# iamwinter/UMPR

Measured on AMD Instinct MI355X. Metric: training samples/sec, higher is better.
Workload: dtype f32

## Files before the change

### include/umpr_hip.h

```cpp
#ifndef UMPR_HIP_H
#define UMPR_HIP_H
#include <stddef.h>
#include <stdint.h>

#ifdef __cplusplus
extern "C" {
#endif

const char* umpr_version(void);
const char* umpr_last_error(void);
int umpr_device_info(int dev, char* name, int name_len, int* compute_units, size_t* hbm_bytes);

int umpr_gemm_f32(const float* A, long lda, int transA, const float* B, long ldb, int transB, float* C, long ldc,
                  int M, int N, int K, const float* bias, int bias_mode, int act, int accumulate, float alpha,
                  float* ws, size_t ws_bytes, void* stream);

int umpr_set_gemm_bf16(int on);

int umpr_set_conv_inference(int on);

int umpr_set_conv_pool_follows(int on);

long umpr_debug_wino_fix_count(void);

int umpr_debug_conv3x3_plan(int pass, int N, int Cin, int Cout, int H, int W, int inference, size_t* ws_bytes, size_t* v_bytes);

int umpr_debug_wino_pool_fold(const float* y, const float* g_pooled, const float* w, const float* x, float* unpooled, float* dx,
                              float* dw, float* db, int N, int Cin, int Cout, int H, int W, int f4, int fold, float* ws,
                              size_t ws_bytes, void* stream);

size_t umpr_embed_gru_bidir_ws_bytes(int N, int L, int E);
int umpr_embed_gru_bidir_fwd(const int64_t* ids, const float* emb, int E,
                             const float* w_ih_f, const float* w_hh_f, const float* b_ih_f, const float* b_hh_f,
                             const float* w_ih_r, const float* w_hh_r, const float* b_ih_r, const float* b_hh_r,
                             const int32_t* lengths, const int32_t* order, const int32_t* dst_row, int N, int L,
                             float* out, float* saved, float* ws, size_t ws_bytes, void* stream);
int umpr_embed_gru_bidir_bwd(const int64_t* ids, const float* emb, int E,
                             const float* w_hh_f, const float* w_hh_r,
                             const int32_t* lengths, const int32_t* order, const int32_t* dst_row, int N, int L,
                             const float* dout, const float* out, const float* saved,
                             float* dw_ih_f, float* dw_hh_f, float* db_ih_f, float* db_hh_f,
                             float* dw_ih_r, float* dw_hh_r, float* db_ih_r, float* db_hh_r,
                             float* ws, size_t ws_bytes, void* stream);

int umpr_embed_gru_bidir_bwd_acc(const int64_t* ids, const float* emb, int E,
                                 const float* w_hh_f, const float* w_hh_r,
                                 const int32_t* lengths, const int32_t* order, const int32_t* dst_row, int N, int L,
                                 const float* dout, const float* out, const float* saved,
                                 float* dw_ih_f, float* dw_hh_f, float* db_ih_f, float* db_hh_f,
                                 float* dw_ih_r, float* dw_hh_r, float* db_ih_r, float* db_hh_r,
                                 int accumulate, float* ws, size_t ws_bytes, void* stream);

// ... 295 lines not shown
```

### umpr_amd/_lib.py

```python
from __future__ import annotations

import ctypes
import os
import threading

import torch

_HERE = os.path.dirname(os.path.abspath(__file__))
LIB_PATH = os.path.join(_HERE, "libumpr_hip.so")

_T = {"p": ctypes.c_void_p, "i": ctypes.c_int, "l": ctypes.c_long, "z": ctypes.c_size_t, "f": ctypes.c_float,
      "d": ctypes.c_double, "u": ctypes.c_uint64}

SIGNATURES = {
    "umpr_version": ("", "s"),
    "umpr_last_error": ("", "s"),
    "umpr_device_info": ("ipipp", "i"),
    "umpr_gemm_f32": ("pliplipliiipiiifpzp", "i"),
    "umpr_embed_gru_bidir_ws_bytes": ("iii", "z"),
    "umpr_embed_gru_bidir_fwd": ("ppipppppppppppiipppzp", "i"),
    "umpr_embed_gru_bidir_bwd": ("ppipppppiippppppppppppzp", "i"),
    "umpr_embed_gru_bidir_bwd_acc": ("ppipppppiipppppppppppipzp", "i"),
    "umpr_embed_gru_bidir_bwd_dx": ("ppipppppiipppppppppppipppipzp", "i"),
    "umpr_embed_grad_chunk": ("", "i"),
# ... 89 lines not shown
    "umpr_feature_fetch_f32": ("pipppiiplpp", "i"),
    "umpr_review_collate": ("pplppppppplpiiiiilpppp", "i"),
    "umpr_review_collate_sampled": ("pplppppppplpiiiiil" "iuil" "pppp", "i"),
    "umpr_bce_head_fwd": ("plpppiipppzp", "i"),
    "umpr_bce_head_bwd": ("plpppppiiplpppzp", "i"),
    "umpr_adam_step": ("ppppldddddldp", "i"),
    "umpr_sq_err_accumulate": ("pplpp", "i"),
    "umpr_adam_step_dev": ("pppplddd" "pp", "i"),
    "umpr_grad_norm_ws_bytes": ("", "z"),
    "umpr_grad_norm": ("ppidfppzpp", "i"),
    "umpr_adam_step_clip": ("ppppldddddld" "pp", "i"),
    "umpr_adam_step_dev_clip": ("pppplddd" "ppp", "i"),
    "umpr_adam_step_groups": ("ppppldddddld" "pp" "ppp" "ii" "p", "i"),
    "umpr_grad_accumulate": ("pppiip", "i"),
    "umpr_ema_update": ("pppidip", "i"),
    "umpr_arena_swap": ("pppip", "i"),
    "umpr_debug_poison_lds": ("pp", "i"),
    "umpr_set_gemm_bf16": ("i", "i"),
    "umpr_set_conv_inference": ("i", "i"),
    "umpr_set_conv_pool_follows": ("i", "i"),
    "umpr_debug_wino_fix_count": ("", "l"),
    "umpr_debug_conv3x3_plan": ("iiiiiiipp", "i"),
    "umpr_debug_wino_pool_fold": ("pppppppp" "iiiiiii" "pzp", "i"),
    "umpr_profile_enable": ("i", "i"),
    "umpr_profile_reset": ("", "i"),
    "umpr_profile_read": ("ippp", "i"),
}


class UmprHipError(RuntimeError):
    pass


class _Tls(threading.local):
    gemm_b16 = False


TLS = _Tls()


class _Lib:
    def __init__(self):
        if not os.path.exists(LIB_PATH):
            raise UmprHipError(
                f"{LIB_PATH} not found: build it with `python -c 'import __graft_entry__ as g; g.build()'` "
                f"(or `make -C umpr_amd/csrc`).  There is no CPU fallback.")
# ... 65 lines not shown
```

### umpr_amd/csrc/api.hip

```cpp
#include <math.h>
#include <stdarg.h>
#include <stdlib.h>

#include <vector>

#include "../../include/umpr_hip.h"
#include "umpr_common.h"
#include "umpr_internal.h"

static thread_local char g_err[512] = "";
void umpr_set_error(const char* fmt, ...) {
  va_list ap;
  va_start(ap, fmt);
  vsnprintf(g_err, sizeof(g_err), fmt, ap);
  va_end(ap);
}

namespace {
const bool g_fc_small = umpr_env_on("UMPR_FC_SMALL");
struct ProfRec { hipEvent_t e0, e1; int family; double work; };
bool g_prof_on = false;
std::vector<ProfRec> g_prof;
std::vector<ProfRec> g_prof_pool;
double g_prof_ms[UMPR_K_COUNT] = {0}, g_prof_work[UMPR_K_COUNT] = {0};
// ... 98 lines not shown
  return p.algo;
}
int umpr_debug_wino_pool_fold(const float* y, const float* g_pooled, const float* w, const float* x, float* unpooled, float* dx,
                              float* dw, float* db, int N, int Cin, int Cout, int H_, int W, int f4, int fold, float* ws,
                              size_t ws_bytes, void* stream) {
  UMPR_REQUIRE(N > 0 && Cin > 0 && Cout > 0 && H_ > 0 && W > 0 && (H_ % 2) == 0 && (W % 2) == 0 && y && g_pooled && ws,
               "debug_wino_pool_fold: bad arguments");
  UMPR_REQUIRE(fold || unpooled, "debug_wino_pool_fold: the un-folded run needs the buffer for the un-pooled gradient");
  UMPR_REQUIRE(!dx || (f4 && w), "debug_wino_pool_fold: the data gradient runs on the 4x4 tile and needs the weights");
  UMPR_REQUIRE(!dw || (x && (!f4 || ((H_ % 4) == 0 && (W % 4) == 0))), "debug_wino_pool_fold: the weight gradient on the 4x4 tile has no edge tiles");
  hipStream_t s = S(stream);
  ConvHints h;
  const float* g = g_pooled;
  if (fold) { h.pooled_dy = true; h.pool_y = y; }
  else {
    if (int rc = umpr_maxpool2_bwd_relu_impl(y, g_pooled, unpooled, (long)N * Cout, H_, W, s)) return rc;
    g = unpooled;
  }
  if (dx)
    if (int rc = umpr_wino_conv3x3(g, w, 1, nullptr, nullptr, dx, N, Cin, Cout, H_, W, 0, ws, ws_bytes / sizeof(float), true, h, s)) return rc;
  if (dw)
    if (int rc = umpr_wino_wgrad(g, x, dw, db, N, Cin, Cout, H_, W, 0, ws, ws_bytes / sizeof(float), f4 != 0, h, s)) return rc;
  return 0;
}

constexpr size_t kSlabs = 256;
namespace {
struct GruWs {
  float *gx, *wslab, *bslab;
  float* kslab; size_t kslab_bytes;
  float *stacked, *rows;
  float *wst, *bst;
  size_t bytes;
};
GruWs gru_ws(float* base, int N, int L, int pitch) {
  Carve c(base, sizeof(float));
  const size_t tiles = umpr_gru_tiles(N);
  GruWs w;
  w.gx = c.take<float>((size_t)N * L * 384); w.wslab = c.take<float>(tiles * 2 * G3 * H); w.bslab = c.take<float>(tiles * 2 * 2 * G3);
  w.wst = c.at<float>(c.off); w.bst = c.at<float>(c.off + (size_t)2 * G3 * pitch * sizeof(float));
  w.kslab_bytes = kSlabs * G3 * pitch * sizeof(float); w.kslab = c.take<float>(kSlabs * G3 * pitch);
  w.stacked = c.take<float>((size_t)2 * G3 * pitch); w.rows = c.take<float>((size_t)N * L * pitch); w.bytes = c.off;
  return w;
}
const bool g_emb_gather = umpr_env_on("UMPR_EMB_GATHER");
__global__ __launch_bounds__(256) void gather_rows_kernel(const int64_t* __restrict__ ids, const float* __restrict__ emb,
// ... 403 lines not shown
}
int umpr_conv3x3_bwd_weight(const float* dy, const float* x, float* dw, float* db, int N, int Cin, int H_, int W,
                            int Cout, float* ws, size_t ws_bytes, void* stream) {
  return umpr_conv3x3_wgrad(dy, x, dw, db, N, Cin, Cout, H_, W, 0, ws, ws_bytes, conv_hints(), S(stream));
}
int umpr_maxpool2_fwd(const float* x, float* y, long planes, int H_, int W, void* stream) {
  return umpr_maxpool2_fwd_impl(x, y, planes, H_, W, S(stream));
}
int umpr_maxpool2_bwd_relu(const float* x, const float* dy, float* dx, long planes, int H_, int W, void* stream) {
  return umpr_maxpool2_bwd_relu_impl(x, dy, dx, planes, H_, W, S(stream));
}

size_t umpr_vgg16_pool5_offset(int n_img) { return vgg_layout(n_img).pool_off[4] * sizeof(float); }

int umpr_vgg16_features_fwd(const float* images, const float* const* params, int n, float* acts, float* ws,
                            size_t ws_bytes, void* stream) {
  UMPR_REQUIRE(n > 0 && images && params && acts, "vgg16_features_fwd: bad arguments");
  UMPR_REQUIRE(ws_bytes >= umpr_vgg16_fwd_ws_bytes(n), "vgg16_features_fwd: workspace too small");
  const VggLayout L = vgg_layout(n);
  hipStream_t s = S(stream);
  const float* x = images;
  int ci = 0;
  for (int b = 0; b < 5; ++b) {
    for (int j = 0; j < kConvPerBlock[b]; ++j, ++ci) {
      float* y = acts + L.conv_off[ci];
      const int hw = L.conv_hw[ci];
      ConvHints hints;
      hints.inference = t_conv_inference;
      hints.pool_follows = j == kConvPerBlock[b] - 1;
      if (L.v_floats[ci] && !hints.inference) { hints.v_slot = acts + L.v_off[ci]; hints.v_slot_floats = L.v_floats[ci]; }
      if (int rc = umpr_conv3x3_run(x, params[2 * ci], 0, params[2 * ci + 1], nullptr, y, n, L.conv_cin[ci], L.conv_cout[ci], hw,
                                    hw, 1, ws, ws_bytes / sizeof(float), hints, s))
        return rc;
      x = y;
    }
    const int hw = L.conv_hw[ci - 1];
    float* y = acts + L.pool_off[b];
    if (int rc = umpr_maxpool2_fwd_impl(x, y, (long)n * kBlockCh[b], hw, hw, s)) return rc;
    x = y;
  }
  return 0;
}

namespace {
struct ClsActs { const float* pool5; float* fc[2]; float* drop[2]; };

int classifier_fwd_impl(const float* const* params, int n, int train, int use_masks, uint64_t seed, const ClsActs& A,
                        uint8_t* masks, float* out, float* ws, size_t ws_bytes, hipStream_t s, int fc_bf16, bool gemm_b16) {
  const float* x = A.pool5;
  for (int j = 0; j < 3; ++j) {
    float* y = j < 2 ? A.fc[j] : out;
    const int act = j < 2 ? UMPR_ACT_RELU : UMPR_ACT_NONE;
    if (g_fc_small && umpr_fc_small_ok(n, kFc[j][1], kFc[j][0])) {
      if (int rc = umpr_fc_small_fwd(x, params[26 + 2 * j], params[27 + 2 * j], y, n, kFc[j][1], kFc[j][0], act, ws,
                                     ws_bytes, s, 0, fc_bf16)) return rc;
    } else {
      UmprGemm g;
      g.A = x; g.lda = kFc[j][0]; g.B = params[26 + 2 * j]; g.ldb = kFc[j][0]; g.transB = true;
      g.C = y; g.ldc = kFc[j][1]; g.M = n; g.N = kFc[j][1]; g.K = kFc[j][0];
      g.bias = params[27 + 2 * j]; g.bias_mode = 1; g.act = act;
      g.split_k = 0; g.ws = ws; g.ws_bytes = ws_bytes; g.b16 = gemm_b16;
// ... 513 lines not shown
```

### umpr_amd/csrc/conv3x3.hip

```cpp
#include "umpr_common.h"
#include "umpr_internal.h"
#include "umpr_tiles.h"
#include <stdlib.h>
#include <type_traits>

namespace {

struct ConvParams {
  const float* x;
  const float* wm;
  const float* bias;
  const float* mask;
  float* y;
  int N, C, H, W, Cout, relu;
  long p0_base;
  long p_end;
};

template <int TM, int TN, bool BIAS, bool MASK, bool TAIL>
__device__ __forceinline__ void igemm_epilogue_as(const f32x16 (&tot)[TM][TN], const ConvParams& p, int HW, int row0,
                                                  const long (&obase)[TN], const bool (&pv)[TN]) {
  const int Cout = p.Cout;
  const bool relu = p.relu != 0;
  float bv[TM][16];
// ... 1101 lines not shown
  }
  if (pass != CONV_DGRAD && !(pass == CONV_FWD && inference) && sw.v_reuse &&
      conv_algo(CONV_FWD, Cin, Cout, H, W, false) == CONV_WINO4 && conv_algo(CONV_WGRAD, Cin, Cout, H, W, false) == CONV_WINO4) {
    const WinoConvGeom fg = umpr_wino_conv_geom(N, Cin, Cout, H, W, true);
    const WinoWgradGeom wg = umpr_wino_wgrad_geom(N, Cin, Cout, H, W, true);
    if (fg.v_floats == (size_t)wg.planes * wg.Cpad * wg.Tpad) p.v_floats = fg.v_floats;
  }
  return p;
}

size_t umpr_conv3x3_pack_floats(int N, int Cin, int Cout, int H, int W) {
  const size_t f = umpr_conv3x3_plan(CONV_FWD, N, Cin, Cout, H, W, false).ws_floats;
  const size_t t = umpr_conv3x3_plan(CONV_DGRAD, N, Cin, Cout, H, W, false).ws_floats;
  return f > t ? f : t;
}

bool umpr_conv3x3_pool_fold_ok(int N, int Cin, int Cout, int H, int W) {
  static const bool on = umpr_env_on("UMPR_POOL_FOLD");
  if (!on || (H % 2) != 0 || (W % 2) != 0) return false;
  const ConvAlgo wg = umpr_conv3x3_plan(CONV_WGRAD, N, Cin, Cout, H, W, false).algo;
  return umpr_conv3x3_plan(CONV_DGRAD, N, Cin, Cout, H, W, false).algo == CONV_WINO4 && (wg == CONV_WINO4 || wg == CONV_WINO2);
}

int umpr_conv3x3_run(const float* x, const float* w, int transposed, const float* bias, const float* mask, float* y,
                     int N, int Cin, int Cout, int H, int W, int relu, float* wpack, size_t wpack_floats,
                     const ConvHints& hints, hipStream_t s) {
  UMPR_REQUIRE(N > 0 && Cin > 0 && H > 0 && W > 0 && Cout > 0, "conv3x3: bad shape");
  UMPR_REQUIRE(transposed || !mask, "conv3x3: the forward pass takes no mask");
  const int M = transposed ? Cin : Cout;
  const int C = transposed ? Cout : Cin;
  const long NP = (long)N * H * W;
  const ConvPlan plan = umpr_conv3x3_plan(transposed ? CONV_DGRAD : CONV_FWD, N, Cin, Cout, H, W, hints.inference);
  ConvAlgo algo = plan.algo;
  const bool fits = wpack && wpack_floats >= plan.ws_floats;
  if (hints.v_slot)
    UMPR_REQUIRE(algo == CONV_WINO4 && fits && plan.v_floats > 0 && plan.v_floats == hints.v_slot_floats,
                 "conv3x3: the V slot does not fit this call (%d -> %d at %dx%d, slot %zu floats, plan %zu)", Cin, Cout, H, W,
                 hints.v_slot_floats, plan.v_floats);
  else if ((algo == CONV_WINO2 || algo == CONV_WINO4) && !fits) algo = plan.direct;
  if (hints.pooled_dy)
    UMPR_REQUIRE(transposed && algo == CONV_WINO4 && hints.pool_y, "conv3x3: no reader with a pooled source for this call (%d -> %d at %dx%d)",
                 Cin, Cout, H, W);
  if (algo == CONV_DIRECT && !wpack) algo = CONV_GENERIC;
  const int family = transposed ? UMPR_K_CONV_DGRAD : UMPR_K_CONV_IGEMM;
  const double work = 2.0 * NP * M * C * 9;
  switch (algo) {
    case CONV_WINO2:
    case CONV_WINO4: {
      UmprProfScope prof(family, work, s);
      return umpr_wino_conv3x3(x, w, transposed, bias, mask, y, N, Cin, Cout, H, W, relu, wpack, wpack_floats,
                               algo == CONV_WINO4, hints, s);
    }
    case CONV_C3: {
      ConvParams p{x, w, bias, nullptr, y, N, Cin, H, W, Cout, relu, 0, NP};
      UmprProfScope prof(family, work, s);
      conv3x3_fwd_c3_kernel<2><<<2048, 256, 0, s>>>(p);
      UMPR_LAUNCH_CHECK("conv3x3_fwd_c3");
      return 0;
    }
    case CONV_DIRECT: {
      const long total = (long)M * ((C + V2_CC - 1) / V2_CC) * V2_KC;
      UMPR_REQUIRE(wpack_floats >= (size_t)total, "conv3x3: weight scratch too small");
      UMPR_REQUIRE(H == W && (W == 224 || W == 112 || W == 56 || W == 28 || W == 14), "conv3x3: the direct kernels need a square VGG map, not %dx%d", H, W);
      int blocks = (int)((total + 255) / 256);
      if (blocks > 4096) blocks = 4096;
// ... 163 lines not shown
```

### umpr_amd/csrc/umpr_internal.h

```cpp
#pragma once
#include <hip/hip_runtime.h>
#include <stdint.h>

struct UmprGemm {
  const float* A = nullptr; long lda = 0; bool transA = false;
  const float* B = nullptr; long ldb = 0; bool transB = false;
  float* C = nullptr; long ldc = 0;
  int M = 0, N = 0, K = 0;
  const int64_t* gatherA = nullptr;
  const int64_t* gatherB = nullptr;
  const float* bias = nullptr; int bias_mode = 0;
  int act = 0; bool accumulate = false; float alpha = 1.0f;
  int split_k = 1;
  float* ws = nullptr; size_t ws_bytes = 0;
  bool b16 = false;
  int winA_L = 0, winA_D = 1, winA_pad = 0;
  int winB_L = 0, winB_D = 1, winB_pad = 0;
};
int umpr_gemm(const UmprGemm& g, hipStream_t stream);
bool umpr_ambient_gemm_b16();

constexpr int D = 128, H = 64, G3 = 192, AT = 64;
bool umpr_merge_small();

// ... 25 lines not shown
  const float* pos_v; const float* neg_v;
  const float* lw; const float* lb;
  const float* fw; const float* fb;
  const float* labels;
  float rate;
  int B, V, P, F;
  float* pred; float* loss;
  float* z;
  float* img_emb; float* pos_match; float* neg_match;
  float* posneg_emb;
  const float* d_loss;
  const float* d_pred;
  float* d_rr; float* d_cu; float* d_ci; float* d_pp; float* d_pn;
  float* d_vgg; float* d_pos_v; float* d_neg_v; float* d_lw; float* d_lb; float* d_fw; float* d_fb;
};
int umpr_head_launch(const UmprHead& p, int backward, hipStream_t s);

enum ConvPass { CONV_FWD = 0, CONV_DGRAD = 1, CONV_WGRAD = 2 };
enum ConvAlgo { CONV_GENERIC = 0 , CONV_C3 = 1 ,
                CONV_DIRECT = 2 , CONV_WINO2 = 3, CONV_WINO4 = 4 };
struct ConvHints {
  bool inference = false, pool_follows = false; float* v_slot = nullptr; size_t v_slot_floats = 0;
  bool pooled_dy = false; const float* pool_y = nullptr;
};
struct ConvPlan {
  ConvAlgo algo;
  ConvAlgo direct;
  bool edge;
  size_t ws_floats;
  size_t v_floats;
};
ConvPlan umpr_conv3x3_plan(ConvPass pass, int N, int Cin, int Cout, int H, int W, bool inference);
size_t umpr_conv3x3_pack_floats(int N, int Cin, int Cout, int H, int W);
bool umpr_conv3x3_pool_fold_ok(int N, int Cin, int Cout, int H, int W);
int umpr_conv3x3_run(const float* x, const float* w, int transposed, const float* bias, const float* mask, float* y,
                     int N, int Cin, int Cout, int H, int W, int relu, float* wpack, size_t wpack_floats,
                     const ConvHints& hints, hipStream_t s);
struct WinoConvGeom { int planes, MT, S; long T, Tpad; bool edge; size_t v_floats, U, V, M, count, tie, floats; };
WinoConvGeom umpr_wino_conv_geom(int N, int C, int M, int H, int W, bool f4);
struct WinoWgradGeom { long T, Tpad; int MT, CT, Mpad, Cpad, stages, splits, stages_per_split, planes, bnc; size_t Gy, V, P, BP, floats; };
WinoWgradGeom umpr_wino_wgrad_geom(int N, int Cin, int Cout, int H, int W, bool f4);
long umpr_wino_last_fix_count();
int umpr_wino_wgrad(const float* dy, const float* x, float* dw, float* db, int N, int Cin, int Cout, int H, int W,
                    int accumulate, float* ws, size_t ws_floats, bool f4, const ConvHints& hints, hipStream_t s);
int umpr_wino_conv3x3(const float* x, const float* w, int transposed, const float* bias, const float* mask, float* y,
                      int N, int Cin, int Cout, int H, int W, int relu, float* ws, size_t ws_floats, bool f4,
                      const ConvHints& hints, hipStream_t s);
int umpr_conv3x3_flip_transpose(const float* w, float* wt, int Cout, int Cin, hipStream_t s);
size_t umpr_conv3x3_wgrad_ws_bytes(int N, int Cin, int Cout, int H, int W);
int umpr_conv3x3_wgrad(const float* gz, const float* x, float* dw, float* db, int N, int Cin, int Cout, int H, int W,
                       int accumulate, float* ws, size_t ws_bytes, const ConvHints& hints, hipStream_t s);
int umpr_maxpool2_fwd_impl(const float* x, float* y, long planes, int H, int W, hipStream_t s);
int umpr_maxpool2_bwd_relu_impl(const float* x, const float* gy, float* gx, long planes, int H, int W, hipStream_t s);

int umpr_wgrad_reduce(const float* slab, const float* bslab, int splits, int Cout, int Cin, float* dw, float* db,
                      int accumulate, hipStream_t s);

struct UmprPF {
  int N, H, W, RW;
  long rows;
  long ptot;
  long lead, tail;
  long ps;
};
UmprPF umpr_pf(int N, int H, int W);
// ... 117 lines not shown
```

### umpr_amd/csrc/winograd.hip

```cpp
#include <type_traits>

#include "umpr_common.h"
#include "umpr_internal.h"

namespace {

constexpr int WK = 32;
constexpr int WBM = 128;
constexpr int WBN = 128;

__device__ __forceinline__ void pool_window_grad(const float2 a, const float2 b, const float gy, float2& ga, float2& gb) {
  int arg = 0;
  float m = a.x;
  if (a.y > m) { m = a.y; arg = 1; }
  if (b.x > m) { m = b.x; arg = 2; }
  if (b.y > m) { m = b.y; arg = 3; }
  const float g = m > 0.f ? gy : 0.f;
  ga = make_float2(arg == 0 ? g : 0.f, arg == 1 ? g : 0.f);
  gb = make_float2(arg == 2 ? g : 0.f, arg == 3 ? g : 0.f);
}
typedef float f32x4_t __attribute__((ext_vector_type(4)));
__device__ __forceinline__ float as_loaded(float v) { asm volatile("" : "+v"(v)); return v; }
__device__ __forceinline__ float4 as_loaded(const float4 v) {
  f32x4_t q = {v.x, v.y, v.z, v.w};
// ... 487 lines not shown
        if (((rows >> (2 * wy)) & 0xFu) != 0xFu) viol |= 1u << (2 * w);
        if (((cols >> (2 * wx)) & 0xFu) != 0xFu) viol |= 2u << (2 * w);
      }
      if (viol & ~bits[t]) atomicOr(&bits[t], viol);
    }
#pragma unroll
    for (int b = 0; b < 6; ++b) {
      float o[6];
      wino4_bt(wc, e[0][b], e[1][b], e[2][b], e[3][b], e[4][b], e[5][b], o);
#pragma unroll
      for (int a = 0; a < 6; ++a) dst[(long)(a * 6 + b) * per] = o[a];
    }
  }
}

struct WinoFix {
  unsigned int* count;
  unsigned int* list;
  unsigned int cap;
  float kappa_eps;
  const unsigned int* tie_bits;
};

template <bool EDGE, bool FIX>
__global__ __launch_bounds__(256) void wino4_output_kernel(const float* __restrict__ Mx, const float* __restrict__ bias,
                                                           const float* __restrict__ mask, float* __restrict__ y, int N,
                                                           int Mch, int H, int W, long Tpad, int Mpad, int relu, Wino4C wc,
                                                           WinoFix fx) {
  const int TH = (H + 3) / 4, TW = (W + 3) / 4;
  const long T = (long)N * TH * TW;
  const long total = (long)Mch * T;
  const long per = (long)Mpad * Tpad;
  for (long i = blockIdx.x * (long)blockDim.x + threadIdx.x; i < total; i += (long)gridDim.x * blockDim.x) {
    const long t = i % T;
    const int m = (int)(i / T);
    const int tx = (int)(t % TW);
    const long r = t / TW;
    const int ty = (int)(r % TH), n = (int)(r / TH);
    const float* src = Mx + (long)m * Tpad + t;
    float am[4][6];
    float as[4][6];
#pragma unroll
    for (int b = 0; b < 6; ++b) {
      float q[6];
#pragma unroll
      for (int a = 0; a < 6; ++a) q[a] = src[(long)(a * 6 + b) * per];
      float o[4];
      wino4_at(wc, q, o);
      am[0][b] = o[0]; am[1][b] = o[1]; am[2][b] = o[2]; am[3][b] = o[3];
      if (FIX) {
#pragma unroll
        for (int a = 0; a < 6; ++a) q[a] = fabsf(q[a]);
        wino4_at_abs(wc, q, o);
        as[0][b] = o[0]; as[1][b] = o[1]; as[2][b] = o[2]; as[3][b] = o[3];
      }
    }
    const float bv = bias ? bias[m] : 0.f;
    const long ob = (((long)n * Mch + m) * H + 4 * ty) * W + 4 * tx;
    float vv[4][4], tau[4][4];
#pragma unroll
    for (int a = 0; a < 4; ++a) {
      float v[4];
      wino4_at(wc, am[a], v);
#pragma unroll
      for (int j = 0; j < 4; ++j) v[j] += bv;
      if (FIX) {
        float sv[4];
        wino4_at_abs(wc, as[a], sv);
#pragma unroll
        for (int j = 0; j < 4; ++j) { vv[a][j] = v[j]; tau[a][j] = fx.kappa_eps * sv[j]; }
      }
      if (relu) {
#pragma unroll
        for (int j = 0; j < 4; ++j) v[j] = fmaxf(v[j], 0.f);
      }
      const long oo = ob + (long)a * W;
      if (EDGE) {
        if (4 * ty + a >= H) continue;
#pragma unroll
        for (int j = 0; j < 4; ++j) {
          if (4 * tx + j < W) {
            float o = v[j];
            if (mask) o = mask[oo + j] > 0.f ? o : 0.f;
            y[oo + j] = o;
          }
        }
        continue;
      }
      if (mask) {
        const float4 mk = *reinterpret_cast<const float4*>(mask + oo);
        v[0] = mk.x > 0.f ? v[0] : 0.f; v[1] = mk.y > 0.f ? v[1] : 0.f;
        v[2] = mk.z > 0.f ? v[2] : 0.f; v[3] = mk.w > 0.f ? v[3] : 0.f;
      }
      *reinterpret_cast<float4*>(y + oo) = make_float4(v[0], v[1], v[2], v[3]);
    }
    if (FIX) {
      unsigned flags = 0;
#pragma unroll
      for (int a = 0; a < 4; ++a)
#pragma unroll
        for (int j = 0; j < 4; ++j)
          if (fabsf(vv[a][j]) < tau[a][j]) flags |= 1u << (4 * a + j);
      if (fx.tie_bits) {
        const unsigned viol = fx.tie_bits[t];
#pragma unroll
        for (int wy = 0; wy < 2; ++wy)
#pragma unroll
          for (int wx = 0; wx < 2; ++wx) {
            float top = 0.f, second = 0.f, tw = 0.f;
            int e1 = 0, e2 = 0;
#pragma unroll
            for (int e = 0; e < 4; ++e) {
              const int a = 2 * wy + (e >> 1), j = 2 * wx + (e & 1);
              const float rv = fmaxf(vv[a][j], 0.f);
              if (rv > top) { second = top; e2 = e1; top = rv; e1 = e; } else if (rv > second) { second = rv; e2 = e; }
              tw = fmaxf(tw, tau[a][j]);
            }
// ... 35 lines not shown
    float acc = 0.f;
    for (int c = lane; c < C; c += 64) {
      const float* xp = x + ((long)n * C + c) * HW;
      const float* wp = w + ((long)m * C + c) * 9;
#pragma unroll
      for (int dy = 0; dy < 3; ++dy) {
        const int py = yy + dy - 1;
        if (py < 0 || py >= H) continue;
#pragma unroll
        for (int dx = 0; dx < 3; ++dx) {
          const int px = xx + dx - 1;
          if (px < 0 || px >= W) continue;
          acc = fmaf(xp[(long)py * W + px], wp[dy * 3 + dx], acc);
        }
      }
    }
#pragma unroll
    for (int o = 32; o > 0; o >>= 1) acc += __shfl_xor(acc, o, 64);
    if (lane == 0) {
      float v = acc + (bias ? bias[m] : 0.f);
      if (relu) v = fmaxf(v, 0.f);
      y[idx] = v;
    }
  }
}

static long wino_tpad(long T) { return (T + WBN - 1) / WBN * WBN; }

struct WinoGemmParams {
  const float* U;
  const float* V;
  float* Mx;
  int MT, S, C;
  long Tpad;
  long TT;
  int Mpad;
  int planes;
};

typedef __attribute__((address_space(3))) void* lds_ptr_t;
template <int FOLD>
__global__ __launch_bounds__(256, 2) void wino_gemm_dma_kernel(WinoGemmParams p) {
  constexpr int SK = WK;
  constexpr int LD = 128;
  constexpr int TM = 2, TN = 2;
  constexpr int KS = SK / 2;
// ... 177 lines not shown
    if (edge) wino4_input_kernel<true, false, true><<<nblk((long)S * WK * TT * WBN, 16384), 256, 0, s>>>(x, V, N, C, S * WK, H, W, Tpad, TT * WBN, wino4_consts(), nullptr, nullptr, hints.pool_y);
    else wino4_input_kernel<false, false, true><<<nblk((long)S * WK * TT * WBN, 16384), 256, 0, s>>>(x, V, N, C, S * WK, H, W, Tpad, TT * WBN, wino4_consts(), nullptr, nullptr, hints.pool_y);
  } else if (f4 && edge) {
    if (tie_bits) wino4_input_kernel<true, true><<<nblk((long)S * WK * TT * WBN, 16384), 256, 0, s>>>(x, V, N, C, S * WK, H, W, Tpad, TT * WBN, wino4_consts(), fx.count, tie_bits);
    else wino4_input_kernel<true, false><<<nblk((long)S * WK * TT * WBN, 16384), 256, 0, s>>>(x, V, N, C, S * WK, H, W, Tpad, TT * WBN, wino4_consts(), fx.count, nullptr);
  } else if (f4) {
    if (tie_bits) wino4_input_kernel<false, true><<<nblk((long)S * WK * TT * WBN, 16384), 256, 0, s>>>(x, V, N, C, S * WK, H, W, Tpad, TT * WBN, wino4_consts(), fx.count, tie_bits);
    else wino4_input_kernel<false, false><<<nblk((long)S * WK * TT * WBN, 16384), 256, 0, s>>>(x, V, N, C, S * WK, H, W, Tpad, TT * WBN, wino4_consts(), fx.count, nullptr);
  }
  else if ((W / 2) % 2 == 0)
    wino_input_pair_kernel<<<nblk((long)S * WK * TT * WBN / 2, 16384), 256, 0, s>>>(x, V, N, C, S * WK, H, W, Tpad, TT * WBN);
  else
    wino_input_kernel<<<nblk((long)S * WK * TT * WBN, 16384), 256, 0, s>>>(x, V, N, C, S * WK, H, W, Tpad, TT * WBN);
  UMPR_LAUNCH_CHECK("wino_input");
  WinoGemmParams p{U, V, Mx, MT, S, C, Tpad, TT, MT * WBM, planes};
  const long groups = (planes * TT + 7) / 8 * 8;
  {
    UmprProfScope prof(UMPR_K_WINO_GEMM, 2.0 * planes * (double)M * C * T, s);
    static const int fold = umpr_env_int("UMPR_WINO_FOLD", 1);
    if (fold == 2) wino_gemm_dma_kernel<2><<<(unsigned)(groups * MT), 256, 0, s>>>(p);
    else wino_gemm_dma_kernel<1><<<(unsigned)(groups * MT), 256, 0, s>>>(p);
  }
  UMPR_LAUNCH_CHECK("wino_gemm");
  if (f4 && fix) {
    if (edge) wino4_output_kernel<true, true><<<nblk((long)M * T, 16384), 256, 0, s>>>(Mx, bias, mask, y, N, M, H, W, Tpad, MT * WBM, relu, wino4_consts(), fx);
    else wino4_output_kernel<false, true><<<nblk((long)M * T, 16384), 256, 0, s>>>(Mx, bias, mask, y, N, M, H, W, Tpad, MT * WBM, relu, wino4_consts(), fx);
    UMPR_LAUNCH_CHECK("wino_output");
    wino_fixup_kernel<<<128, 256, 0, s>>>(x, w, bias, y, fx.list, fx.count, fx.cap, C, M, H, W, relu);
    UMPR_LAUNCH_CHECK("wino_fixup");
    t_last_fix_count = fx.count;
    return 0;
  }
  if (f4 && edge)
    wino4_output_kernel<true, false><<<nblk((long)M * T, 16384), 256, 0, s>>>(Mx, bias, mask, y, N, M, H, W, Tpad, MT * WBM, relu, wino4_consts(), fx);
  else if (f4)
    wino4_output_kernel<false, false><<<nblk((long)M * T, 16384), 256, 0, s>>>(Mx, bias, mask, y, N, M, H, W, Tpad, MT * WBM, relu, wino4_consts(), fx);
  else if ((W / 2) % 2 == 0)
    wino_output_pair_kernel<<<nblk((long)M * T / 2, 16384), 256, 0, s>>>(Mx, bias, mask, y, N, M, H, W, Tpad, MT * WBM, relu);
  else
    wino_output_kernel<<<nblk((long)M * T, 16384), 256, 0, s>>>(Mx, bias, mask, y, N, M, H, W, Tpad, MT * WBM, relu);
  UMPR_LAUNCH_CHECK("wino_output");
  return 0;
}

namespace {

template <bool POOL>
__global__ void wino_dy_kernel(const float* __restrict__ dy, float* __restrict__ Gy, int N, int Mch, int H, int W,
                               long Tpad, long Tw, int Mpad, const float* __restrict__ pool_y) {
  const int TH = H / 2, TW = W / 2;
  const long T = (long)N * TH * TW;
  const long total = (long)Mch * Tw;
  const long per = (long)Mpad * Tpad;
  for (long i = blockIdx.x * (long)blockDim.x + threadIdx.x; i < total; i += (long)gridDim.x * blockDim.x) {
    const long t = i % Tw;
    const int m = (int)(i / Tw);
    float* dst = Gy + (long)m * Tpad + t;
    if (t >= T) {
#pragma unroll
// ... 283 lines not shown
  __shared__ float outs[64 * 9];
  if (g == 0 && ok) {
#pragma unroll
    for (int a = 0; a < 36; ++a) v[a] = ((v[a] + red[0][a][cl]) + red[1][a][cl]) + red[2][a][cl];
    float gv[3][6];
#pragma unroll
    for (int b = 0; b < 6; ++b) {
      float o[3];
      wino4_gt(wc, v + b, 6, o);
      gv[0][b] = o[0]; gv[1][b] = o[1]; gv[2][b] = o[2];
    }
#pragma unroll
    for (int a = 0; a < 3; ++a) {
      float o[3];
      wino4_gt(wc, gv[a], 1, o);
      outs[cl * 9 + a * 3 + 0] = o[0]; outs[cl * 9 + a * 3 + 1] = o[1]; outs[cl * 9 + a * 3 + 2] = o[2];
    }
  }
  __syncthreads();
  const int c0 = (blockIdx.x % chunks) * 64;
  const int nout = (C - c0 < 64 ? C - c0 : 64) * 9;
  float* d = dw + ((long)m * C + c0) * 9;
  for (int i = threadIdx.x; i < nout; i += 256) d[i] = accumulate ? d[i] + outs[i] : outs[i];
}

struct WinoWgradParams {
  const float* Gy;
  const float* V;
  float* P;
  int MT, CT, Mpad, Cpad;
  long Tpad;
  int stages;
  int stages_per_split;
  int planes;
};

constexpr int WLDK = WK + 4;

template <int TN>
__global__ __launch_bounds__(256, 2) void wino_wgrad_gemm_kernel(WinoWgradParams p) {
  constexpr int LD = WLDK;
  constexpr int TM = 2;
  constexpr int BNC = 64 * TN;
  constexpr int NG = WK / 8;
  constexpr int SFLUSH = 4;
  __shared__ __attribute__((aligned(16))) float As[2][WBM * LD];
// ... 128 lines not shown
    float gv[3][4];
#pragma unroll
    for (int b = 0; b < 4; ++b) {
      gv[0][b] = v[0][b] + 0.5f * (v[1][b] + v[2][b]);
      gv[1][b] = 0.5f * (v[1][b] - v[2][b]);
      gv[2][b] = 0.5f * (v[1][b] + v[2][b]) + v[3][b];
    }
    float* d = dw + i * 9;
#pragma unroll
    for (int a = 0; a < 3; ++a) {
      const float o0 = gv[a][0] + 0.5f * (gv[a][1] + gv[a][2]);
      const float o1 = 0.5f * (gv[a][1] - gv[a][2]);
      const float o2 = 0.5f * (gv[a][1] + gv[a][2]) + gv[a][3];
      if (accumulate) { d[a * 3 + 0] += o0; d[a * 3 + 1] += o1; d[a * 3 + 2] += o2; }
      else { d[a * 3 + 0] = o0; d[a * 3 + 1] = o1; d[a * 3 + 2] = o2; }
    }
  }
}

constexpr int kWinoWgradTargetWgs = 1024;
static const int g_wino_wgrad_rounds = umpr_env_int("UMPR_WINO_WGRAD_ROUNDS", 1);
}

WinoWgradGeom umpr_wino_wgrad_geom(int N, int Cin, int Cout, int H, int W, bool f4) {
  WinoWgradGeom g;
  g.planes = f4 ? 36 : 16;
  g.T = f4 ? (long)N * ((H + 3) / 4) * ((W + 3) / 4) : (long)N * (H / 2) * (W / 2);
  g.Tpad = wino_tpad(g.T);
  g.bnc = Cin <= 64 ? 64 : WBN;
  g.MT = (Cout + WBM - 1) / WBM; g.CT = (Cin + g.bnc - 1) / g.bnc;
  g.Mpad = g.MT * WBM; g.Cpad = g.CT * g.bnc;
  g.stages = (int)(g.Tpad / WK);
  const int tiles = g.planes * g.MT * g.CT;
  const int max_splits = g.stages / 8 > 0 ? g.stages / 8 : 1;
  int splits = (kWinoWgradTargetWgs + tiles - 1) / tiles;
  if (g_wino_wgrad_rounds && (long)tiles * max_splits >= 512) {
    double best = 0.0;
    const int hi = max_splits < splits ? max_splits : splits;
    for (int sp = 1; sp <= hi; ++sp) {
      const long wgs = (long)tiles * sp;
      if (wgs < 512) continue;
      const double eff = (double)wgs / (double)((wgs + 511) / 512 * 512);
      if (eff > best) best = eff;
    }
    for (int sp = 1; sp <= hi; ++sp) {
      const long wgs = (long)tiles * sp;
// ... 38 lines not shown
    else wino_dy_kernel<false><<<nblk((long)Cout * g.Tpad, 16384), 256, 0, s>>>(dy, Gy, N, Cout, H, W, g.Tpad, g.Tpad, g.Mpad, nullptr);
  }
  UMPR_LAUNCH_CHECK("wino_dy");
  if (hints.v_slot) {
    UMPR_REQUIRE(f4 && !edge && hints.v_slot_floats == (size_t)g.planes * g.Cpad * g.Tpad,
                 "winograd wgrad: the V slot does not match this layer (%d -> %d at %dx%d)", Cin, Cout, H, W);
    V = hints.v_slot;
  } else if (f4 && edge)
    wino4_input_kernel<true, false><<<nblk((long)g.Cpad * g.Tpad, 16384), 256, 0, s>>>(x, V, N, Cin, g.Cpad, H, W, g.Tpad, g.Tpad, wino4_consts(), nullptr, nullptr);
  else if (f4)
    wino4_input_kernel<false, false><<<nblk((long)g.Cpad * g.Tpad, 16384), 256, 0, s>>>(x, V, N, Cin, g.Cpad, H, W, g.Tpad, g.Tpad, wino4_consts(), nullptr, nullptr);
  else if ((W / 2) % 2 == 0)
    wino_input_pair_kernel<<<nblk((long)g.Cpad * g.Tpad / 2, 16384), 256, 0, s>>>(x, V, N, Cin, g.Cpad, H, W, g.Tpad, g.Tpad);
  else
    wino_input_kernel<<<nblk((long)g.Cpad * g.Tpad, 16384), 256, 0, s>>>(x, V, N, Cin, g.Cpad, H, W, g.Tpad, g.Tpad);
  UMPR_LAUNCH_CHECK("wino_input(wgrad)");
  WinoWgradParams p{Gy, V, P, g.MT, g.CT, g.Mpad, g.Cpad, g.Tpad, g.stages, g.stages_per_split, g.planes};
  {
    UmprProfScope prof(UMPR_K_WINO_WGRAD_GEMM, 2.0 * g.planes * (double)Cout * Cin * g.T, s);
    if (g.bnc == 64) wino_wgrad_gemm_kernel<1><<<(unsigned)(g.planes * g.MT * g.CT * g.splits), 256, 0, s>>>(p);
    else wino_wgrad_gemm_kernel<2><<<(unsigned)(g.planes * g.MT * g.CT * g.splits), 256, 0, s>>>(p);
  }
  UMPR_LAUNCH_CHECK("wino_wgrad_gemm");
  if (f4)
    wino4_wgrad_finish_kernel<<<(unsigned)((long)Cout * ((Cin + 63) / 64)), 256, 0, s>>>(P, g.splits, Cout, Cin, g.Mpad, g.Cpad, dw,
                                                                                     accumulate, wino4_consts());
  else if (g.splits >= 8)
    wino_wgrad_finish_wide_kernel<<<(unsigned)((long)Cout * ((Cin + 63) / 64)), 256, 0, s>>>(P, g.splits, Cout, Cin, g.Mpad, g.Cpad,
                                                                                         dw, accumulate);
  else
    wino_wgrad_finish_kernel<<<nblk((long)Cout * Cin, 4096), 256, 0, s>>>(P, g.splits, Cout, Cin, g.Mpad, g.Cpad, dw, accumulate);
  UMPR_LAUNCH_CHECK("wino_wgrad_finish");
  if (fused_bias) {
    wino_bias_sum_waves_kernel<<<(unsigned)((Cout + 3) / 4), 256, 0, s>>>(BP, db, Cout, g.Tpad / 64, accumulate);
    UMPR_LAUNCH_CHECK("wino_bias_sum_waves");
  } else if (db) {
    UMPR_REQUIRE((size_t)N * Cout <= (size_t)g.splits * g.planes * g.Mpad * g.Cpad && ((long)H * W) % 4 == 0,
                 "winograd wgrad: bias-gradient scratch");
    if (pooled) wino_bias_part_wave_kernel<true><<<(unsigned)(((long)N * Cout + 3) / 4), 256, 0, s>>>(dy, P, (long)H * W, (long)N * Cout, py, W);
    else wino_bias_part_wave_kernel<false><<<(unsigned)(((long)N * Cout + 3) / 4), 256, 0, s>>>(dy, P, (long)H * W, (long)N * Cout, nullptr, W);
    UMPR_LAUNCH_CHECK("wino_bias_part");
    wino_bias_sum_kernel<<<(Cout + 255) / 256, 256, 0, s>>>(P, db, N, Cout, accumulate);
    UMPR_LAUNCH_CHECK("wino_bias_sum");
  }
  return 0;
}
```

Measured before the change: 2164.

## Fuse maxpool into Winograd forward output and widen wgrad finish kernel

Adds an optional path where the 4x4-tile Winograd forward output kernel also writes the 2x2 max-pooled result, with a fixup pass that recomputes pooled values touched by corrected outputs. This would skip the separate maxpool launch and its re-read of the activation, but it is gated behind the UMPR_FWD_FOLD environment variable. Separately, the f4 weight-gradient finish now always uses a new 1024-thread kernel that splits the reduction over splits across 16 waves, staging partial sums in shared memory before the transform. The new finish kernel aims for more memory parallelism in the split reduction, at the cost of more shared memory and a fixed summation order.

```diff
diff --git a/include/umpr_hip.h b/include/umpr_hip.h
--- a/include/umpr_hip.h
+++ b/include/umpr_hip.h
@@ -28,6 +28,12 @@
 int umpr_debug_wino_pool_fold(const float* y, const float* g_pooled, const float* w, const float* x, float* unpooled, float* dx,
                               float* dw, float* db, int N, int Cin, int Cout, int H, int W, int f4, int fold, float* ws,
                               size_t ws_bytes, void* stream);
+
+int umpr_debug_wino_fwd_fold(const float* x, const float* w, const float* bias, float* y, float* pooled, int N, int Cin, int Cout,
+                             int H, int W, int inference, int fold, float* ws, size_t ws_bytes, void* stream);
+
+int umpr_debug_wino4_wgrad_finish(const float* P, int splits, int Cout, int Cin, int Mpad, int Cpad, float* dw, int accumulate,
+                                  int former, void* stream);
 
 size_t umpr_embed_gru_bidir_ws_bytes(int N, int L, int E);
 int umpr_embed_gru_bidir_fwd(const int64_t* ids, const float* emb, int E,
diff --git a/umpr_amd/_lib.py b/umpr_amd/_lib.py
--- a/umpr_amd/_lib.py
+++ b/umpr_amd/_lib.py
@@ -135,6 +135,8 @@
     "umpr_debug_wino_fix_count": ("", "l"),
     "umpr_debug_conv3x3_plan": ("iiiiiiipp", "i"),
     "umpr_debug_wino_pool_fold": ("pppppppp" "iiiiiii" "pzp", "i"),
+    "umpr_debug_wino_fwd_fold": ("ppppp" "iiiiiii" "pzp", "i"),
+    "umpr_debug_wino4_wgrad_finish": ("p" "iiiii" "p" "ii" "p", "i"),
     "umpr_profile_enable": ("i", "i"),
     "umpr_profile_reset": ("", "i"),
     "umpr_profile_read": ("ippp", "i"),
diff --git a/umpr_amd/csrc/api.hip b/umpr_amd/csrc/api.hip
--- a/umpr_amd/csrc/api.hip
+++ b/umpr_amd/csrc/api.hip
@@ -144,6 +144,23 @@
   if (dw)
     if (int rc = umpr_wino_wgrad(g, x, dw, db, N, Cin, Cout, H_, W, 0, ws, ws_bytes / sizeof(float), f4 != 0, h, s)) return rc;
   return 0;
+}
+
+int umpr_debug_wino_fwd_fold(const float* x, const float* w, const float* bias, float* y, float* pooled, int N, int Cin, int Cout,
+                             int H_, int W, int inference, int fold, float* ws, size_t ws_bytes, void* stream) {
+  UMPR_REQUIRE(N > 0 && Cin > 0 && Cout > 0 && H_ > 0 && W > 0 && (H_ % 2) == 0 && (W % 2) == 0 && x && w && y && pooled && ws,
+               "debug_wino_fwd_fold: bad arguments");
+  hipStream_t s = S(stream);
+  ConvHints h;
+  h.inference = inference != 0; h.pool_follows = true;
+  if (fold) h.pool_out = pooled;
+  if (int rc = umpr_wino_conv3x3(x, w, 0, bias, nullptr, y, N, Cin, Cout, H_, W, 1, ws, ws_bytes / sizeof(float), true, h, s)) return rc;
+  return fold ? 0 : umpr_maxpool2_fwd_impl(y, pooled, (long)N * Cout, H_, W, s);
+}
+int umpr_debug_wino4_wgrad_finish(const float* P, int splits, int Cout, int Cin, int Mpad, int Cpad, float* dw, int accumulate,
+                                  int former, void* stream) {
+  UMPR_REQUIRE(P && dw && splits > 0 && Cout > 0 && Cin > 0 && Mpad >= Cout && Cpad >= Cin, "debug_wino4_wgrad_finish: bad arguments");
+  return umpr_wino4_wgrad_finish_launch(P, splits, Cout, Cin, Mpad, Cpad, dw, accumulate, former != 0, S(stream));
 }
 
 constexpr size_t kSlabs = 256;
@@ -593,6 +610,7 @@
   const float* x = images;
   int ci = 0;
   for (int b = 0; b < 5; ++b) {
+    bool pooled = false;
     for (int j = 0; j < kConvPerBlock[b]; ++j, ++ci) {
       float* y = acts + L.conv_off[ci];
       const int hw = L.conv_hw[ci];
@@ -600,6 +618,10 @@
       hints.inference = t_conv_inference;
       hints.pool_follows = j == kConvPerBlock[b] - 1;
       if (L.v_floats[ci] && !hints.inference) { hints.v_slot = acts + L.v_off[ci]; hints.v_slot_floats = L.v_floats[ci]; }
+      if (hints.pool_follows && umpr_conv3x3_fwd_fold_ok(n, L.conv_cin[ci], L.conv_cout[ci], hw, hw, hints.inference)) {
+        hints.pool_out = acts + L.pool_off[b];
+        pooled = true;
+      }
       if (int rc = umpr_conv3x3_run(x, params[2 * ci], 0, params[2 * ci + 1], nullptr, y, n, L.conv_cin[ci], L.conv_cout[ci], hw,
                                     hw, 1, ws, ws_bytes / sizeof(float), hints, s))
         return rc;
@@ -607,7 +629,8 @@
     }
     const int hw = L.conv_hw[ci - 1];
     float* y = acts + L.pool_off[b];
-    if (int rc = umpr_maxpool2_fwd_impl(x, y, (long)n * kBlockCh[b], hw, hw, s)) return rc;
+    if (!pooled)
+      if (int rc = umpr_maxpool2_fwd_impl(x, y, (long)n * kBlockCh[b], hw, hw, s)) return rc;
     x = y;
   }
   return 0;
diff --git a/umpr_amd/csrc/conv3x3.hip b/umpr_amd/csrc/conv3x3.hip
--- a/umpr_amd/csrc/conv3x3.hip
+++ b/umpr_amd/csrc/conv3x3.hip
@@ -1147,6 +1147,11 @@
   return umpr_conv3x3_plan(CONV_DGRAD, N, Cin, Cout, H, W, false).algo == CONV_WINO4 && (wg == CONV_WINO4 || wg == CONV_WINO2);
 }
 
+bool umpr_conv3x3_fwd_fold_ok(int N, int Cin, int Cout, int H, int W, bool inference) {
+  static const bool on = umpr_env_on("UMPR_FWD_FOLD");
+  return on && (H % 2) == 0 && (W % 2) == 0 && umpr_conv3x3_plan(CONV_FWD, N, Cin, Cout, H, W, inference).algo == CONV_WINO4;
+}
+
 int umpr_conv3x3_run(const float* x, const float* w, int transposed, const float* bias, const float* mask, float* y,
                      int N, int Cin, int Cout, int H, int W, int relu, float* wpack, size_t wpack_floats,
                      const ConvHints& hints, hipStream_t s) {
@@ -1166,6 +1171,9 @@
   if (hints.pooled_dy)
     UMPR_REQUIRE(transposed && algo == CONV_WINO4 && hints.pool_y, "conv3x3: no reader with a pooled source for this call (%d -> %d at %dx%d)",
                  Cin, Cout, H, W);
+  if (hints.pool_out)
+    UMPR_REQUIRE(!transposed && algo == CONV_WINO4, "conv3x3: no kernel that pools its output for this call (%d -> %d at %dx%d)",
+                 Cin, Cout, H, W);
   if (algo == CONV_DIRECT && !wpack) algo = CONV_GENERIC;
   const int family = transposed ? UMPR_K_CONV_DGRAD : UMPR_K_CONV_IGEMM;
   const double work = 2.0 * NP * M * C * 9;
diff --git a/umpr_amd/csrc/umpr_internal.h b/umpr_amd/csrc/umpr_internal.h
--- a/umpr_amd/csrc/umpr_internal.h
+++ b/umpr_amd/csrc/umpr_internal.h
@@ -71,6 +71,7 @@
 struct ConvHints {
   bool inference = false, pool_follows = false; float* v_slot = nullptr; size_t v_slot_floats = 0;
   bool pooled_dy = false; const float* pool_y = nullptr;
+  float* pool_out = nullptr;
 };
 struct ConvPlan {
   ConvAlgo algo;
@@ -82,6 +83,7 @@
 ConvPlan umpr_conv3x3_plan(ConvPass pass, int N, int Cin, int Cout, int H, int W, bool inference);
 size_t umpr_conv3x3_pack_floats(int N, int Cin, int Cout, int H, int W);
 bool umpr_conv3x3_pool_fold_ok(int N, int Cin, int Cout, int H, int W);
+bool umpr_conv3x3_fwd_fold_ok(int N, int Cin, int Cout, int H, int W, bool inference);
 int umpr_conv3x3_run(const float* x, const float* w, int transposed, const float* bias, const float* mask, float* y,
                      int N, int Cin, int Cout, int H, int W, int relu, float* wpack, size_t wpack_floats,
                      const ConvHints& hints, hipStream_t s);
@@ -90,6 +92,8 @@
 struct WinoWgradGeom { long T, Tpad; int MT, CT, Mpad, Cpad, stages, splits, stages_per_split, planes, bnc; size_t Gy, V, P, BP, floats; };
 WinoWgradGeom umpr_wino_wgrad_geom(int N, int Cin, int Cout, int H, int W, bool f4);
 long umpr_wino_last_fix_count();
+int umpr_wino4_wgrad_finish_launch(const float* P, int splits, int Cout, int Cin, int Mpad, int Cpad, float* dw, int accumulate,
+                                   bool former, hipStream_t s);
 int umpr_wino_wgrad(const float* dy, const float* x, float* dw, float* db, int N, int Cin, int Cout, int H, int W,
                     int accumulate, float* ws, size_t ws_floats, bool f4, const ConvHints& hints, hipStream_t s);
 int umpr_wino_conv3x3(const float* x, const float* w, int transposed, const float* bias, const float* mask, float* y,
diff --git a/umpr_amd/csrc/winograd.hip b/umpr_amd/csrc/winograd.hip
--- a/umpr_amd/csrc/winograd.hip
+++ b/umpr_amd/csrc/winograd.hip
@@ -533,11 +533,11 @@
   const unsigned int* tie_bits;
 };
 
-template <bool EDGE, bool FIX>
+template <bool EDGE, bool FIX, bool POOL = false>
 __global__ __launch_bounds__(256) void wino4_output_kernel(const float* __restrict__ Mx, const float* __restrict__ bias,
                                                            const float* __restrict__ mask, float* __restrict__ y, int N,
                                                            int Mch, int H, int W, long Tpad, int Mpad, int relu, Wino4C wc,
-                                                           WinoFix fx) {
+                                                           WinoFix fx, float* __restrict__ pool_out = nullptr) {
   const int TH = (H + 3) / 4, TW = (W + 3) / 4;
   const long T = (long)N * TH * TW;
   const long total = (long)Mch * T;
@@ -569,6 +569,7 @@
     const float bv = bias ? bias[m] : 0.f;
     const long ob = (((long)n * Mch + m) * H + 4 * ty) * W + 4 * tx;
     float vv[4][4], tau[4][4];
+    float st[4][4];
 #pragma unroll
     for (int a = 0; a < 4; ++a) {
       float v[4];
@@ -594,6 +595,7 @@
             float o = v[j];
             if (mask) o = mask[oo + j] > 0.f ? o : 0.f;
             y[oo + j] = o;
+            if (POOL) st[a][j] = o;
           }
         }
         continue;
@@ -604,6 +606,24 @@
         v[2] = mk.z > 0.f ? v[2] : 0.f; v[3] = mk.w > 0.f ? v[3] : 0.f;
       }
       *reinterpret_cast<float4*>(y + oo) = make_float4(v[0], v[1], v[2], v[3]);
+      if (POOL) { st[a][0] = v[0]; st[a][1] = v[1]; st[a][2] = v[2]; st[a][3] = v[3]; }
+    }
+    if (POOL) {
+      const int PW = W / 2;
+      const long pb = (((long)n * Mch + m) * (H / 2) + 2 * ty) * PW + 2 * tx;
+#pragma unroll
+      for (int wy = 0; wy < 2; ++wy) {
+        if (EDGE && 4 * ty + 2 * wy >= H) continue;
+        const float p0 = fmaxf(fmaxf(st[2 * wy][0], st[2 * wy][1]), fmaxf(st[2 * wy + 1][0], st[2 * wy + 1][1]));
+        if (EDGE) {
+          pool_out[pb + (long)wy * PW] = p0;
+          if (4 * tx + 2 < W)
+            pool_out[pb + (long)wy * PW + 1] = fmaxf(fmaxf(st[2 * wy][2], st[2 * wy][3]), fmaxf(st[2 * wy + 1][2], st[2 * wy + 1][3]));
+        } else {
+          const float p1 = fmaxf(fmaxf(st[2 * wy][2], st[2 * wy][3]), fmaxf(st[2 * wy + 1][2], st[2 * wy + 1][3]));
+          *reinterpret_cast<float2*>(pool_out + pb + (long)wy * PW) = make_float2(p0, p1);
+        }
+      }
     }
     if (FIX) {
       unsigned flags = 0;
@@ -685,6 +705,24 @@
       if (relu) v = fmaxf(v, 0.f);
       y[idx] = v;
     }
+  }
+}
+
+__global__ __launch_bounds__(256) void wino_fixup_pool_kernel(const float* __restrict__ y, float* __restrict__ pool_out,
+                                                              const unsigned int* __restrict__ list,
+                                                              const unsigned int* __restrict__ count, unsigned cap, int H, int W) {
+  const unsigned n_fix = min(*count, cap);
+  const int PW = W / 2, PH = H / 2;
+  for (unsigned i = blockIdx.x * blockDim.x + threadIdx.x; i < n_fix; i += gridDim.x * blockDim.x) {
+    const unsigned idx = list[i];
+    const int xo = (int)(idx % W) >> 1;
+    const unsigned r = idx / W;
+    const int yo = (int)(r % H) >> 1;
+    const long pl = r / H;
+    const float* s = y + (pl * H + 2 * yo) * W + 2 * xo;
+    const float2 a = *reinterpret_cast<const float2*>(s);
+    const float2 b = *reinterpret_cast<const float2*>(s + W);
+    pool_out[(pl * PH + yo) * PW + xo] = fmaxf(fmaxf(a.x, a.y), fmaxf(b.x, b.y));
   }
 }
 
@@ -908,19 +946,32 @@
     else wino_gemm_dma_kernel<1><<<(unsigned)(groups * MT), 256, 0, s>>>(p);
   }
   UMPR_LAUNCH_CHECK("wino_gemm");
+  float* const pool = hints.pool_out;
+  if (pool) UMPR_REQUIRE(f4 && !transposed && (reinterpret_cast<uintptr_t>(pool) & 7) == 0, "winograd: the pooled output needs a forward on the 4x4 tile");
+  const unsigned ogrid = nblk((long)M * T, 16384);
   if (f4 && fix) {
-    if (edge) wino4_output_kernel<true, true><<<nblk((long)M * T, 16384), 256, 0, s>>>(Mx, bias, mask, y, N, M, H, W, Tpad, MT * WBM, relu, wino4_consts(), fx);
-    else wino4_output_kernel<false, true><<<nblk((long)M * T, 16384), 256, 0, s>>>(Mx, bias, mask, y, N, M, H, W, Tpad, MT * WBM, relu, wino4_consts(), fx);
+    if (edge && pool) wino4_output_kernel<true, true, true><<<ogrid, 256, 0, s>>>(Mx, bias, mask, y, N, M, H, W, Tpad, MT * WBM, relu, wino4_consts(), fx, pool);
+    else if (edge) wino4_output_kernel<true, true><<<ogrid, 256, 0, s>>>(Mx, bias, mask, y, N, M, H, W, Tpad, MT * WBM, relu, wino4_consts(), fx);
+    else if (pool) wino4_output_kernel<false, true, true><<<ogrid, 256, 0, s>>>(Mx, bias, mask, y, N, M, H, W, Tpad, MT * WBM, relu, wino4_consts(), fx, pool);
+    else wino4_output_kernel<false, true><<<ogrid, 256, 0, s>>>(Mx, bias, mask, y, N, M, H, W, Tpad, MT * WBM, relu, wino4_consts(), fx);
     UMPR_LAUNCH_CHECK("wino_output");
     wino_fixup_kernel<<<128, 256, 0, s>>>(x, w, bias, y, fx.list, fx.count, fx.cap, C, M, H, W, relu);
     UMPR_LAUNCH_CHECK("wino_fixup");
+    if (pool) {
+      wino_fixup_pool_kernel<<<128, 256, 0, s>>>(y, pool, fx.list, fx.count, fx.cap, H, W);
+      UMPR_LAUNCH_CHECK("wino_fixup_pool");
+    }
     t_last_fix_count = fx.count;
     return 0;
   }
-  if (f4 && edge)
-    wino4_output_kernel<true, false><<<nblk((long)M * T, 16384), 256, 0, s>>>(Mx, bias, mask, y, N, M, H, W, Tpad, MT * WBM, relu, wino4_consts(), fx);
+  if (f4 && edge && pool)
+    wino4_output_kernel<true, false, true><<<ogrid, 256, 0, s>>>(Mx, bias, mask, y, N, M, H, W, Tpad, MT * WBM, relu, wino4_consts(), fx, pool);
+  else if (f4 && edge)
+    wino4_output_kernel<true, false><<<ogrid, 256, 0, s>>>(Mx, bias, mask, y, N, M, H, W, Tpad, MT * WBM, relu, wino4_consts(), fx);
+  else if (f4 && pool)
+    wino4_output_kernel<false, false, true><<<ogrid, 256, 0, s>>>(Mx, bias, mask, y, N, M, H, W, Tpad, MT * WBM, relu, wino4_consts(), fx, pool);
   else if (f4)
-    wino4_output_kernel<false, false><<<nblk((long)M * T, 16384), 256, 0, s>>>(Mx, bias, mask, y, N, M, H, W, Tpad, MT * WBM, relu, wino4_consts(), fx);
+    wino4_output_kernel<false, false><<<ogrid, 256, 0, s>>>(Mx, bias, mask, y, N, M, H, W, Tpad, MT * WBM, relu, wino4_consts(), fx);
   else if ((W / 2) % 2 == 0)
     wino_output_pair_kernel<<<nblk((long)M * T / 2, 16384), 256, 0, s>>>(Mx, bias, mask, y, N, M, H, W, Tpad, MT * WBM, relu);
   else
@@ -1250,6 +1301,88 @@
   const int nout = (C - c0 < 64 ? C - c0 : 64) * 9;
   float* d = dw + ((long)m * C + c0) * 9;
   for (int i = threadIdx.x; i < nout; i += 256) d[i] = accumulate ? d[i] + outs[i] : outs[i];
+}
+
+struct Wino4GtPinned {
+  struct Site { int o0, o1, o2; };
+  static constexpr Site first(int b) {
+    return b == 0 ? Site{0, 0, 2} : b == 1 ? Site{1, 0, 1} : b == 2 ? Site{1, 1, 1} : Site{0, 1, 2};
+  }
+  static constexpr Site second(int a) {
+    return a == 1 ? Site{2, 0, 1} : Site{0, 1, 2};
+  }
+};
+__device__ __forceinline__ void wino4_gt_pinned(const Wino4C& c, const float* __restrict__ v, float d34, Wino4GtPinned::Site s,
+                                                float& o0, float& o1, float& o2) {
+#pragma clang fp contract(off)
+  const float s12 = v[1] + v[2], d12 = v[1] - v[2], s34 = v[3] + v[4];
+  const float t = s.o0 == 1 ? __builtin_fmaf(c.ca, s12, c.g0 * v[0]) : __builtin_fmaf(c.g0, v[0], c.ca * s12);
+  o0 = s.o0 == 2 ? t + c.cb * s34 : __builtin_fmaf(c.cb, s34, t);
+  const float A = c.ca * c.a, B = c.cb * c.b;
+  o1 = s.o1 == 0 ? A * d12 + B * d34 : s.o1 == 1 ? __builtin_fmaf(A, d12, B * d34) : __builtin_fmaf(B, d34, A * d12);
+  const float A2 = c.ca * c.a2, B2 = c.cb * c.b2;
+  o2 = (s.o2 == 1 ? __builtin_fmaf(A2, s12, B2 * s34) : __builtin_fmaf(B2, s34, A2 * s12)) + v[5];
+}
+
+__global__ __launch_bounds__(1024) void wino4_wgrad_finish_stream_kernel(const float* __restrict__ P, int splits, int Mch, int C,
+                                                                         int Mpad, int Cpad, float* __restrict__ dw, int accumulate,
+                                                                         Wino4C wc) {
+  __shared__ float part[4][36][64];
+  __shared__ float outs[64 * 9];
+  const int cl = threadIdx.x & 63, wave = threadIdx.x >> 6;
+  const int g = wave & 3, pq = wave >> 2;
+  const int chunks = (C + 63) / 64;
+  const int m = blockIdx.x / chunks, c = (blockIdx.x % chunks) * 64 + cl;
+  const long per = (long)Mpad * Cpad;
+  const bool ok = c < C;
+  float acc[9];
+#pragma unroll
+  for (int k = 0; k < 9; ++k) acc[k] = 0.f;
+  if (ok) {
+    const float* src = P + (long)(pq * 9) * per + (long)m * Cpad + c;
+    int sp = g;
+    for (; sp + 4 < splits; sp += 8) {
+      float t0[9], t1[9];
+#pragma unroll
+      for (int k = 0; k < 9; ++k) t0[k] = src[((long)sp * 36 + k) * per];
+#pragma unroll
+      for (int k = 0; k < 9; ++k) t1[k] = src[((long)(sp + 4) * 36 + k) * per];
+#pragma unroll
+      for (int k = 0; k < 9; ++k) { acc[k] += t0[k]; acc[k] += t1[k]; }
+    }
+    if (sp < splits) {
+#pragma unroll
+      for (int k = 0; k < 9; ++k) acc[k] += src[((long)sp * 36 + k) * per];
+    }
+  }
+#pragma unroll
+  for (int k = 0; k < 9; ++k) part[g][pq * 9 + k][cl] = acc[k];
+  __syncthreads();
+  if (wave == 0 && ok) {
+    float gv[3][6];
+    float gv03 = 0.f;
+#pragma unroll
+    for (int b = 0; b < 6; ++b) {
+      float col[6];
+#pragma unroll
+      for (int a = 0; a < 6; ++a)
+        col[a] = ((part[0][a * 6 + b][cl] + part[1][a * 6 + b][cl]) + part[2][a * 6 + b][cl]) + part[3][a * 6 + b][cl];
+      const Wino4GtPinned::Site f = Wino4GtPinned::first(b);
+      wino4_gt_pinned(wc, col, col[3] - col[4], f, gv[0][b], gv[1][b], gv[2][b]);
+      if (b == 3) { float u1, u2; wino4_gt_pinned(wc, col, col[3] - col[4], {1, f.o1, f.o2}, gv03, u1, u2); }
+    }
+#pragma unroll
+    for (int a = 0; a < 3; ++a) {
+      float o[3];
+      wino4_gt_pinned(wc, gv[a], (a == 0 ? gv03 : gv[a][3]) - gv[a][4], Wino4GtPinned::second(a), o[0], o[1], o[2]);
+      outs[cl * 9 + a * 3 + 0] = o[0]; outs[cl * 9 + a * 3 + 1] = o[1]; outs[cl * 9 + a * 3 + 2] = o[2];
+    }
+  }
+  __syncthreads();
+  const int c0 = (blockIdx.x % chunks) * 64;
+  const int nout = (C - c0 < 64 ? C - c0 : 64) * 9;
+  float* d = dw + ((long)m * C + c0) * 9;
+  for (int i = threadIdx.x; i < nout; i += 1024) d[i] = accumulate ? d[i] + outs[i] : outs[i];
 }
 
 struct WinoWgradParams {
@@ -1424,6 +1557,15 @@
 static const int g_wino_wgrad_rounds = umpr_env_int("UMPR_WINO_WGRAD_ROUNDS", 1);
 }
 
+int umpr_wino4_wgrad_finish_launch(const float* P, int splits, int Cout, int Cin, int Mpad, int Cpad, float* dw, int accumulate,
+                                   bool former, hipStream_t s) {
+  const unsigned grid = (unsigned)((long)Cout * ((Cin + 63) / 64));
+  if (former) wino4_wgrad_finish_kernel<<<grid, 256, 0, s>>>(P, splits, Cout, Cin, Mpad, Cpad, dw, accumulate, wino4_consts());
+  else wino4_wgrad_finish_stream_kernel<<<grid, 1024, 0, s>>>(P, splits, Cout, Cin, Mpad, Cpad, dw, accumulate, wino4_consts());
+  UMPR_LAUNCH_CHECK("wino_wgrad_finish");
+  return 0;
+}
+
 WinoWgradGeom umpr_wino_wgrad_geom(int N, int Cin, int Cout, int H, int W, bool f4) {
   WinoWgradGeom g;
   g.planes = f4 ? 36 : 16;
@@ -1508,10 +1650,9 @@
     else wino_wgrad_gemm_kernel<2><<<(unsigned)(g.planes * g.MT * g.CT * g.splits), 256, 0, s>>>(p);
   }
   UMPR_LAUNCH_CHECK("wino_wgrad_gemm");
-  if (f4)
-    wino4_wgrad_finish_kernel<<<(unsigned)((long)Cout * ((Cin + 63) / 64)), 256, 0, s>>>(P, g.splits, Cout, Cin, g.Mpad, g.Cpad, dw,
-                                                                                     accumulate, wino4_consts());
-  else if (g.splits >= 8)
+  if (f4) {
+    if (int rc = umpr_wino4_wgrad_finish_launch(P, g.splits, Cout, Cin, g.Mpad, g.Cpad, dw, accumulate, false, s)) return rc;
+  } else if (g.splits >= 8)
     wino_wgrad_finish_wide_kernel<<<(unsigned)((long)Cout * ((Cin + 63) / 64)), 256, 0, s>>>(P, g.splits, Cout, Cin, g.Mpad, g.Cpad,
                                                                                          dw, accumulate);
   else
```

After: 2158. No clear change (-0.2%).
